# amirkdv/biseqt

Hardware: AMD Instinct MI355X
Metric: GCUPS (DP cell updates/s) banded local align (higher is better)
Workload: dtype i16

## Files before the change

biseqt_amd/csrc/pw_device.h:

```cpp
#ifndef PW_DEVICE_H
#define PW_DEVICE_H

#include <hip/hip_runtime.h>
#include <stdint.h>

#define PW_FN __device__ __forceinline__
#include "pw_wave.h"
#include "pw_launch.h"

namespace pw {

PW_FN uint32_t dev_shl1_in(uint32_t m, bool flag) {
  const uint64_t mask = __builtin_amdgcn_ballot_w64(flag);
  uint32_t r;
  uint64_t cout;
  asm("v_addc_co_u32 %0, %1, %2, %2, %3" : "=v"(r), "=s"(cout) : "v"(m), "s"(mask));
  return r;
}

template <typename T, bool ALWAYS_LDS> PW_FN T dev_tab_read(const T* tab, uint32_t handle, uint32_t off, bool in_lds) {
  typedef __attribute__((address_space(3))) const T lds_T;
  if (ALWAYS_LDS || in_lds) return *(lds_T*)(uintptr_t)(handle + off);
  return *(const T*)((const char*)tab + off);
}
PW_FN uint32_t dev_lds_handle(const void* p) {
  return (uint32_t)(uintptr_t)(__attribute__((address_space(3))) const char*)p;
}

PW_FN uint32_t dev_const_dword(const uint8_t* base, int idx) {
  typedef const __attribute__((address_space(4))) uint32_t c_u32;
  return ((c_u32*)base)[idx];
}

struct DevP {
  PW_FN static uint32_t const_dword(const uint8_t* base, int idx) { return dev_const_dword(base, idx); }
  template <typename T, bool A> PW_FN static T tab_read(const T* tab, uint32_t h, uint32_t off, bool in_lds) { return dev_tab_read<T, A>(tab, h, off, in_lds); }
  PW_FN static uint32_t shl1_in(uint32_t m, bool flag) { return dev_shl1_in(m, flag); }
  PW_FN static int lane() { return (int)(threadIdx.x & 63u); }
  PW_FN static int32_t shr1(int32_t v, int32_t old) {
    return __builtin_amdgcn_update_dpp(old, v, 0x138 , 0xf, 0xf, false);
  }
  PW_FN static int32_t shl1(int32_t v, int32_t old) {
    return __builtin_amdgcn_update_dpp(old, v, 0x130 , 0xf, 0xf, false);
  }
  PW_FN static int32_t shr1z(int32_t v) { return __builtin_amdgcn_update_dpp(0, v, 0x138 , 0xf, 0xf, true); }
  PW_FN static int32_t shl1z(int32_t v) { return __builtin_amdgcn_update_dpp(0, v, 0x130 , 0xf, 0xf, true); }
  PW_FN static int32_t shfl_xor(int32_t v, int m) { return __shfl_xor(v, m, 64); }
  PW_FN static int32_t uniform(int32_t v) { return __builtin_amdgcn_readfirstlane(v); }
  PW_FN static int nlanes() { return 64; }
  PW_FN static int nwaves() { return 1; }
  PW_FN static int32_t wave_bcast(int32_t v, int) { return v; }
  PW_FN static int lane0() { return 0; }
  PW_FN static bool central() { return true; }
  static constexpr bool kVirtualLanes = false;
  static constexpr bool kBatchedShifts = false;
};

template <int N, int MAXW> PW_FN void wg_shift_right(int32_t* v, const int32_t* old, int phase) {
  __shared__ int32_t edge[2][MAXW][N];
  const int w = (int)(threadIdx.x >> 6), l = (int)(threadIdx.x & 63u);
  int32_t r[N];
#pragma unroll
  for (int i = 0; i < N; i++) r[i] = __builtin_amdgcn_update_dpp(old[i], v[i], 0x138 , 0xf, 0xf, false);
  if (l == 63) {
#pragma unroll
    for (int i = 0; i < N; i++) edge[phase][w][i] = v[i];
  }
  asm volatile("s_waitcnt lgkmcnt(0)\n\ts_barrier" ::: "memory");
  if (l == 0 && w > 0) {
#pragma unroll
    for (int i = 0; i < N; i++) r[i] = edge[phase][w - 1][i];
  }
#pragma unroll
  for (int i = 0; i < N; i++) v[i] = r[i];
}
template <int N, int MAXW> PW_FN void wg_shift_left(int32_t* v, const int32_t* old, int phase) {
  __shared__ int32_t edge[2][MAXW][N];
  const int w = (int)(threadIdx.x >> 6), l = (int)(threadIdx.x & 63u), nw = (int)(blockDim.x >> 6);
  int32_t r[N];
#pragma unroll
  for (int i = 0; i < N; i++) r[i] = __builtin_amdgcn_update_dpp(old[i], v[i], 0x130 , 0xf, 0xf, false);
  if (l == 0) {
#pragma unroll
    for (int i = 0; i < N; i++) edge[phase][w][i] = v[i];
  }
  asm volatile("s_waitcnt lgkmcnt(0)\n\ts_barrier" ::: "memory");
  if (l == 63 && w + 1 < nw) {
#pragma unroll
    for (int i = 0; i < N; i++) r[i] = edge[phase][w + 1][i];
  }
#pragma unroll
  for (int i = 0; i < N; i++) v[i] = r[i];
}

struct DevPM {
  PW_FN static uint32_t const_dword(const uint8_t* base, int idx) { return dev_const_dword(base, idx); }
  template <typename T, bool A> PW_FN static T tab_read(const T* tab, uint32_t h, uint32_t off, bool in_lds) { return dev_tab_read<T, A>(tab, h, off, in_lds); }
  PW_FN static uint32_t shl1_in(uint32_t m, bool flag) { return dev_shl1_in(m, flag); }
  PW_FN static int lane() { return (int)threadIdx.x; }
  PW_FN static int lane0() { return 0; }
  PW_FN static bool central() { return true; }
  static constexpr bool kVirtualLanes = false;
  static constexpr bool kBatchedShifts = true;
  template <int N> PW_FN static void shrv(int32_t* v, const int32_t* old, int phase) { wg_shift_right<N, 16>(v, old, phase); }
  template <int N> PW_FN static void shlv(int32_t* v, const int32_t* old, int phase) { wg_shift_left<N, 16>(v, old, phase); }
  PW_FN static int nlanes() { return (int)blockDim.x; }
  PW_FN static int nwaves() { return (int)(blockDim.x >> 6); }
  PW_FN static int32_t shr1(int32_t v, int32_t old) {
    __shared__ int32_t edge[16];
    const int w = (int)(threadIdx.x >> 6), l = (int)(threadIdx.x & 63u);
    int32_t r = __builtin_amdgcn_update_dpp(old, v, 0x138 , 0xf, 0xf, false);
    if (l == 63) edge[w] = v;
    __syncthreads();
    if (l == 0 && w > 0) r = edge[w - 1];
    __syncthreads();
    return r;
  }
  PW_FN static int32_t shl1(int32_t v, int32_t old) {
    __shared__ int32_t edge[16];
    const int w = (int)(threadIdx.x >> 6), l = (int)(threadIdx.x & 63u);
    int32_t r = __builtin_amdgcn_update_dpp(old, v, 0x130 , 0xf, 0xf, false);
    if (l == 0) edge[w] = v;
    __syncthreads();
    if (l == 63 && w + 1 < (int)(blockDim.x >> 6)) r = edge[w + 1];
    __syncthreads();
    return r;
  }
  PW_FN static int32_t shfl_xor(int32_t v, int m) { return __shfl_xor(v, m, 64); }
  PW_FN static int32_t uniform(int32_t v) { return __builtin_amdgcn_readfirstlane(v); }
  PW_FN static int32_t wave_bcast(int32_t v, int w) {
    __shared__ int32_t slot[16];
    if ((threadIdx.x & 63u) == 0) slot[threadIdx.x >> 6] = v;
    __syncthreads();
    const int32_t r = slot[w];
    __syncthreads();
    return r;
  }
};

constexpr int kMaxLdsL = 32;

#ifndef PW_FILL_ATTR
#define PW_FILL_ATTR
#endif
template <typename T, int BK, bool BANY, bool TRACK, bool GENERIC>
__global__ __launch_bounds__(64) PW_FILL_ATTR void k_fill(const FillParams<T> a) {
  constexpr bool TAB = true;
  __shared__ T sub_lds[TAB ? kMaxLdsL * kMaxLdsL : 1];
  const T* tab = a.subst;
  if (TAB) {
    if (a.L <= kMaxLdsL) {
      for (int i = (int)threadIdx.x; i < a.L * a.L; i += 64) sub_lds[i] = a.subst[i];
      __syncthreads();
      tab = sub_lds;
    }
  }
  const int slot = (int)blockIdx.x;
  const int pair = a.order ? a.order[slot] : slot;
  const PairDesc pd = a.pairs[pair];
  WaveFill<DevP, T, BK, BANY, TRACK, GENERIC> w(a, pd, tab);
  w.tab_handle = dev_lds_handle(sub_lds); w.tab_in_lds = tab == sub_lds;
  w.pair_slot = pair;
  w.run();
}

#ifndef PW_FILL16_WAVES
#define PW_FILL16_WAVES 0
#endif
#ifndef PW_FILL16_WAVES_SEG
#define PW_FILL16_WAVES_SEG 0
#endif
template <int BK, bool SEG, int RULE> struct Fill16Occupancy {
  static constexpr unsigned w = SEG ? PW_FILL16_WAVES_SEG : PW_FILL16_WAVES;
  static constexpr unsigned lo = w ? w : 1, hi = w ? w : 8;
};
template <int BK, bool SEG, int RULE, bool MAT = false>
__global__ __launch_bounds__(64) PW_FILL_ATTR
__attribute__((amdgpu_waves_per_eu(Fill16Occupancy<BK, SEG, RULE>::lo, Fill16Occupancy<BK, SEG, RULE>::hi)))
void k_fill16(const FillParams<int32_t> a) {
  const WaveDesc wd = a.waves[blockIdx.x];
  WaveFill16<DevP, BK, SEG, RULE, MAT> w(a, wd);
  w.run();
}

template <int BK, int RULE, bool MAT = false>
__global__ __launch_bounds__(512) void k_fill16_mw(const FillParams<int32_t> a) {
  const WaveDesc wd = a.waves[blockIdx.x];
  WaveFill16<DevPM, BK, false, RULE, MAT> w(a, wd);
  w.run();
}

constexpr int kTileLanes = PW_TILE_LANES, kTileGhost = PW_TILE_GHOST, kTileCentral = kTileLanes - 2 * kTileGhost;
struct DevPT {
  PW_FN static uint32_t const_dword(const uint8_t* base, int idx) { return dev_const_dword(base, idx); }
  template <typename T, bool A> PW_FN static T tab_read(const T* tab, uint32_t h, uint32_t off, bool in_lds) { return dev_tab_read<T, A>(tab, h, off, in_lds); }
  PW_FN static uint32_t shl1_in(uint32_t m, bool flag) { return dev_shl1_in(m, flag); }
  PW_FN static int tile() {
#ifdef PW_TILE_NO_XCD_REMAP
    return (int)blockIdx.x;
#else
    return (int)(blockIdx.x & 7u) * (int)(gridDim.x >> 3) + (int)(blockIdx.x >> 3);
#endif
  }
  PW_FN static int lane0() { return tile() * kTileCentral - kTileGhost; }
  PW_FN static int lane() { return lane0() + (int)threadIdx.x; }
  PW_FN static int nlanes() { return lane0() + kTileLanes; }
  PW_FN static int nwaves() { return kTileLanes / 64; }
  PW_FN static bool central() { return (int)threadIdx.x >= kTileGhost && (int)threadIdx.x < kTileLanes - kTileGhost; }
  static constexpr bool kVirtualLanes = true;
  static constexpr bool kBatchedShifts = true;
  template <int N> PW_FN static void shrv(int32_t* v, const int32_t* old, int phase) { wg_shift_right<N, kTileLanes / 64>(v, old, phase); }
  template <int N> PW_FN static void shlv(int32_t* v, const int32_t* old, int phase) { wg_shift_left<N, kTileLanes / 64>(v, old, phase); }
  PW_FN static void wg_max4(int (&v)[4]) {
    __shared__ int red[4];
    if (threadIdx.x < 4) red[threadIdx.x] = -0x7fffffff;
    __syncthreads();
#pragma unroll
    for (int i = 0; i < 4; i++) atomicMax(&red[i], v[i]);
    __syncthreads();
#pragma unroll
    for (int i = 0; i < 4; i++) v[i] = red[i];
  }
  PW_FN static int32_t shr1(int32_t v, int32_t old) {
    __shared__ int32_t edge[kTileLanes / 64];
    const int w = (int)(threadIdx.x >> 6), l = (int)(threadIdx.x & 63u);
    int32_t r = __builtin_amdgcn_update_dpp(old, v, 0x138 , 0xf, 0xf, false);
    if (l == 63) edge[w] = v;
    __syncthreads();
    if (l == 0 && w > 0) r = edge[w - 1];
    __syncthreads();
    return r;
  }
  PW_FN static int32_t shl1(int32_t v, int32_t old) {
    __shared__ int32_t edge[kTileLanes / 64];
    const int w = (int)(threadIdx.x >> 6), l = (int)(threadIdx.x & 63u);
    int32_t r = __builtin_amdgcn_update_dpp(old, v, 0x130 , 0xf, 0xf, false);
    if (l == 0) edge[w] = v;
    __syncthreads();
    if (l == 63 && w + 1 < kTileLanes / 64) r = edge[w + 1];
    __syncthreads();
    return r;
  }
  PW_FN static int32_t shfl_xor(int32_t v, int m) { return __shfl_xor(v, m, 64); }
  PW_FN static int32_t uniform(int32_t v) { return __builtin_amdgcn_readfirstlane(v); }
  PW_FN static int32_t wave_bcast(int32_t v, int) { return v; }
};
// ... 138 lines not shown
```

biseqt_amd/csrc/pw_wave.h:

```cpp
#ifndef PW_WAVE_H
#define PW_WAVE_H

#ifndef PW_FN
#error "PW_FN must be defined by the includer"
#endif

#include "pw_types.h"
#if !defined(__HIPCC__)
#include <stdlib.h>
#endif

namespace pw {

template <typename T> struct ScoreTraits;
template <> struct ScoreTraits<int32_t> {
  static constexpr bool is_int = true;
  PW_FN static int32_t neg() { return -(1 << 28); }
  PW_FN static int32_t zero_blk() { return 0; }
  PW_FN static int32_t max2(int32_t a, int32_t b) { return a > b ? a : b; }
  PW_FN static int32_t gap_offer(bool kept, int32_t go, int32_t A) { return kept ? A : A + go; }
};
template <> struct ScoreTraits<double> {
  static constexpr bool is_int = false;
  PW_FN static double neg() { return -1.0e300; }
// ... 452 lines not shown
      const int ox = P::shfl_xor(cx, off), oy = P::shfl_xor(cy, off), oh = P::shfl_xor(hv, off);
      const bool take = oh && (!hv || os > cs || (os == cs && ok_ < ck));
      if (take) { cs = os; ck = ok_; cx = ox; cy = oy; hv = 1; }
    }
    if (P::nwaves() > 1) {
      T bs = cs; uint64_t bk_ = ck; int bx = cx, by = cy, bh = 0;
      for (int wv = 0; wv < P::nwaves(); wv++) {
        const T os = xwave_bcast<P>(cs, wv);
        const uint64_t ok_ = xwave_bcast<P>(ck, wv);
        const int ox = P::wave_bcast(cx, wv), oy = P::wave_bcast(cy, wv), oh = P::wave_bcast(hv, wv);
        const bool take = oh && (!bh || os > bs || (os == bs && ok_ < bk_));
        if (take) { bs = os; bk_ = ok_; bx = ox; by = oy; bh = 1; }
      }
      cs = bs; ck = bk_; cx = bx; cy = by; hv = bh;
    }
    if (lane == 0) {
      Result r;
      r.score = (double)cs * a.score_mul;
      r.opt_i = a.banded ? cx - cy - pd.dmin : cx;
      r.opt_j = a.banded ? (cx < cy ? cx : cy) : cy;
      r.origin_idx = 0; r.mutant_idx = 0; r.tx_len = 0; r.status = 0;
      if (!hv || (endrule == END_STD_LOCAL && !(cs > T(0)))) { r.opt_i = -1; r.opt_j = -1; r.score = 0.0; }
      a.results[pair_slot] = r;
    }
  }
  int pair_slot;
};

struct __attribute__((aligned(8))) U4 { uint32_t x, y, z, w; };
struct __attribute__((packed)) PackedU64 { uint64_t v; };
struct __attribute__((packed)) PackedU32 { uint32_t v; };

namespace pk {
#if defined(__HIP_DEVICE_COMPILE__)
typedef short s2_t __attribute__((ext_vector_type(2)));
typedef unsigned short u2_t __attribute__((ext_vector_type(2)));
PW_FN s2_t as_s2(uint32_t v) { return __builtin_bit_cast(s2_t, v); }
PW_FN u2_t as_u2(uint32_t v) { return __builtin_bit_cast(u2_t, v); }
PW_FN uint32_t add(uint32_t a, uint32_t b) { return __builtin_bit_cast(uint32_t, (u2_t)(as_u2(a) + as_u2(b))); }
PW_FN uint32_t sub(uint32_t a, uint32_t b) { return __builtin_bit_cast(uint32_t, (u2_t)(as_u2(a) - as_u2(b))); }
PW_FN uint32_t add32(uint32_t a, uint32_t b) { return a + b; }
PW_FN uint32_t subsat(uint32_t a, uint32_t b) { return __builtin_bit_cast(uint32_t, __builtin_elementwise_sub_sat(as_u2(a), as_u2(b))); }
PW_FN uint32_t max(uint32_t a, uint32_t b) { return __builtin_bit_cast(uint32_t, __builtin_elementwise_max(as_s2(a), as_s2(b))); }
PW_FN uint32_t minu(uint32_t a, uint32_t b) { return __builtin_bit_cast(uint32_t, __builtin_elementwise_min(as_u2(a), as_u2(b))); }
PW_FN uint32_t maxu(uint32_t a, uint32_t b) { return __builtin_bit_cast(uint32_t, __builtin_elementwise_max(as_u2(a), as_u2(b))); }
PW_FN uint32_t shru(uint32_t a, uint32_t sh) { return __builtin_bit_cast(uint32_t, (u2_t)(as_u2(a) >> as_u2(sh))); }
PW_FN uint32_t mad(uint32_t a, uint32_t b, uint32_t c) { return __builtin_bit_cast(uint32_t, (u2_t)(as_u2(a) * as_u2(b) + as_u2(c))); }
PW_FN uint32_t mins(uint32_t a, uint32_t b) { return __builtin_bit_cast(uint32_t, __builtin_elementwise_min(as_s2(a), as_s2(b))); }
PW_FN uint32_t align16(uint32_t hi, uint32_t lo) { return __builtin_amdgcn_alignbit(hi, lo, 16); }
PW_FN uint32_t sign(uint32_t a, uint32_t sh15) { return __builtin_bit_cast(uint32_t, (s2_t)(as_s2(a) >> as_s2(sh15))); }
PW_FN uint32_t opaque(uint32_t v) { asm volatile("" : "+v"(v)); return v; }
PW_FN uint32_t opaque_su(uint32_t v) { asm volatile("" : "+s"(v)); return v; }
PW_FN uint8_t* opaque_s(uint8_t* v) { asm volatile("" : "+s"(v)); return v; }
PW_FN void store_global(uint8_t* base, uint32_t off, const U4& v) {
  typedef __attribute__((address_space(1))) uint8_t gbyte_t;
  typedef __attribute__((address_space(1))) U4 gu4_t;
  *(gu4_t*)((gbyte_t*)base + off) = v;
}
PW_FN uint32_t perm(uint32_t a, uint32_t b, uint32_t sel) { return __builtin_amdgcn_perm(a, b, sel); }
#else
PW_FN uint32_t mk(uint32_t lo, uint32_t hi) { return (lo & 0xffffu) | (hi << 16); }
PW_FN int32_t sl(uint32_t v) { return (int16_t)(v & 0xffffu); }
PW_FN int32_t sh(uint32_t v) { return (int16_t)(v >> 16); }
PW_FN uint32_t add(uint32_t a, uint32_t b) { return mk((a & 0xffffu) + (b & 0xffffu), (a >> 16) + (b >> 16)); }
PW_FN uint32_t sub(uint32_t a, uint32_t b) { return mk((a & 0xffffu) - (b & 0xffffu), (a >> 16) - (b >> 16)); }
#if !defined(__HIPCC__)
inline unsigned& add32_breaches() { static unsigned n = 0; return n; }
PW_FN uint32_t add32(uint32_t a, uint32_t b) {
  if ((a & 0xffffu) >= 0xff80u || (a >> 16) >= 0xff80u) add32_breaches()++;
  return a + b;
}
#else
PW_FN uint32_t add32(uint32_t a, uint32_t b) { return a + b; }
#endif
PW_FN uint32_t subsat(uint32_t a, uint32_t b) {
  const uint32_t al = a & 0xffffu, bl = b & 0xffffu, ah = a >> 16, bh = b >> 16;
  return mk(al > bl ? al - bl : 0u, ah > bh ? ah - bh : 0u);
}
PW_FN uint32_t max(uint32_t a, uint32_t b) { return mk((uint32_t)(sl(a) > sl(b) ? sl(a) : sl(b)), (uint32_t)(sh(a) > sh(b) ? sh(a) : sh(b))); }
PW_FN uint32_t minu(uint32_t a, uint32_t b) {
  const uint32_t al = a & 0xffffu, bl = b & 0xffffu, ah = a >> 16, bh = b >> 16;
  return mk(al < bl ? al : bl, ah < bh ? ah : bh);
}
PW_FN uint32_t mad(uint32_t a, uint32_t b, uint32_t c) {
  return mk((uint32_t)(sl(a) * sl(b) + sl(c)), (uint32_t)(sh(a) * sh(b) + sh(c)));
}
PW_FN uint32_t maxu(uint32_t a, uint32_t b) {
  const uint32_t al = a & 0xffffu, bl = b & 0xffffu, ah = a >> 16, bh = b >> 16;
  return mk(al > bl ? al : bl, ah > bh ? ah : bh);
}
PW_FN uint32_t shru(uint32_t a, uint32_t sh) { return mk((a & 0xffffu) >> (sh & 0xfu), (a >> 16) >> ((sh >> 16) & 0xfu)); }
PW_FN uint32_t mins(uint32_t a, uint32_t b) { return mk((uint32_t)(sl(a) < sl(b) ? sl(a) : sl(b)), (uint32_t)(sh(a) < sh(b) ? sh(a) : sh(b))); }
PW_FN uint32_t align16(uint32_t hi, uint32_t lo) { return (lo >> 16) | (hi << 16); }
PW_FN uint32_t sign(uint32_t a, uint32_t) { return mk(sl(a) < 0 ? 0xffffu : 0u, sh(a) < 0 ? 0xffffu : 0u); }
PW_FN uint32_t opaque(uint32_t v) { return v; }
PW_FN uint32_t opaque_su(uint32_t v) { return v; }
PW_FN uint8_t* opaque_s(uint8_t* v) { return v; }
PW_FN void store_global(uint8_t* base, uint32_t off, const U4& v) { *(U4*)(base + off) = v; }
PW_FN uint32_t perm(uint32_t a, uint32_t b, uint32_t sel) {
  const uint64_t in = ((uint64_t)a << 32) | b;
  uint32_t r = 0;
  for (int i = 0; i < 4; i++) {
    const uint32_t c = (sel >> (8 * i)) & 0xffu;
    uint32_t v;
    if (c >= 13) v = 0xffu;
    else if (c == 12) v = 0u;
    else if (c >= 8) v = ((in >> (8 * (2 * (c - 8) + 1) + 7)) & 1u) ? 0xffu : 0u;
    else v = (uint32_t)(in >> (8 * c)) & 0xffu;
    r |= v << (8 * i);
  }
  return r;
}
#endif
PW_FN uint32_t both(int32_t v) { return ((uint32_t)v & 0xffffu) | ((uint32_t)v << 16); }
PW_FN uint32_t pack(int32_t lo, int32_t hi) { return ((uint32_t)lo & 0xffffu) | ((uint32_t)hi << 16); }
PW_FN int32_t lo_s(uint32_t v) { return (int32_t)(int16_t)(v & 0xffffu); }
PW_FN int32_t hi_s(uint32_t v) { return (int32_t)(int16_t)(v >> 16); }
}
#if !defined(__HIPCC__)
extern "C" __attribute__((used, visibility("default"))) inline unsigned pw_pk_add32_breaches(int reset) {
  const unsigned n = pk::add32_breaches();
  if (reset) pk::add32_breaches() = 0;
  return n;
}
namespace pk {
inline unsigned* ramp_block_counts() { static unsigned n[4] = {0, 0, 0, 0}; return n; }
inline int& ramp_free_emu() { static int v = -1; return v; }
}
extern "C" __attribute__((used, visibility("default"))) inline void pw_ramp_block_counts(unsigned* out, int reset) {
  for (int i = 0; i < 4; i++) { out[i] = pk::ramp_block_counts()[i]; if (reset) pk::ramp_block_counts()[i] = 0; }
}
extern "C" __attribute__((used, visibility("default"))) inline void pw_emu_ramp_free(int v) { pk::ramp_free_emu() = v; }
#endif

template <class P, int BK, bool SEG, int RULE = 0, bool MAT = false>
struct WaveFill16 {
  static constexpr bool SC4 = RULE == 3;
  static constexpr int RL = SC4 ? 0 : RULE;
  static constexpr int SCL = SC4 ? 4 : 1;
  static constexpr bool ANYB = RL == 0 || RL == 4;
  static constexpr bool TRK = RL == 0 || RL == 5;
  static constexpr bool CAP = !TRK;
  static_assert(BK % 4 == 0, "packed layout needs an even number of cells per step");
  static constexpr int R = BK / 2;
  static constexpr int RH = R / 2;
#ifdef PW_FILL16_UNR
  static constexpr int UNR = PW_FILL16_UNR;
#else
  static constexpr int UNR = BK <= 8 ? 4 : (BK <= 16 ? 2 : 1);
#endif
  static constexpr int32_t NEG16 = ANYB ? -8192 : -24000;
  static constexpr uint32_t SENT_O = 0xfffeu, SENT_M = 0xffffu;
  static constexpr uint32_t MSEL = 0x0c00u, MOUT = 8u;
  static constexpr bool FIXSEL = MAT && RH == 2;
  PW_FN static uint32_t sel4_fed(int it) { return ((uint32_t)it >> 1) & 1u; }
  PW_FN static bool sel4_lo(int k, int p) { return (((k + 7 - p) >> 1) & 1) != 0; }
  using Base = WaveFill<P, int32_t, BK, true, true, false>;

  const FillParams<int32_t>& a;
  const WaveDesc wd;
  PairDesc pd;
  int li;
  bool valid, segfirst, seglast;
  int pair_slot;
  const uint8_t* oseq;
  const uint8_t* mseq;
  int X, Y, ndiag, owlast, mwlast, xfeed_o, yfeed_m;
  uint32_t fo_lo, fo_hi, fm_lo, fm_hi, fo_n0, fo_n1, fo_n2, fm_n0, fm_n1, fm_n2;

  uint32_t HE[RH], UE[RH], LE[RH], HO[RH], UO[RH], LO[RH];
  uint32_t bestE[RH], bestO[RH], btE[RH], btO[RH];
  uint32_t gebE[RH], gebO[RH];
  uint32_t clE[RH], clO[RH];
  uint32_t tfE[RH], tfO[RH], tlE[RH], tlO[RH];
  uint32_t accE[RH], accO[RH], acc2E[RH], acc2O[RH];
  uint32_t OW[RH], MW[RH];
  uint32_t ROW[MAT ? R : 1];
  uint32_t BIASV, MADJ;
  uint32_t MR0, MR1, MR2, MR3;
  uint32_t ONE, SH15, C2, C4, C16, NDELTA, MATCHV, GOV, GOVI, NEGV, LIMV;
  uint32_t kbE[RH], kbO[RH], C8, SEVEN;
  uint32_t up_prev;
  uint32_t left_next;
  int phase_l, phase_r;
  uint32_t mrow0, mrow_step, mspare, mgroup;
  static constexpr bool SPLIT = ANYB && MAT;
  static constexpr bool KEPT = SC4 && SPLIT;
  static constexpr bool SBASE = !SEG && SPLIT;
  static constexpr bool RAMPF = SPLIT && TRK;
  bool rf;
  uint32_t flimx, flimy;
  uint32_t mrowb;
  uint8_t* mbase[BK / 4];

  PW_FN WaveFill16(const FillParams<int32_t>& a_, const WaveDesc& wd_) : a(a_), wd(wd_) {}

  template <int EK>
  PW_FN void cellpair(uint32_t& Hs, uint32_t& Us, uint32_t& Ls, uint32_t& bests, uint32_t& bts, uint32_t geb,
                      uint32_t tf, uint32_t tl, uint32_t& acc, uint32_t up, uint32_t left, uint32_t oc,
                      uint32_t mc, uint32_t tv, uint32_t clampL = 0, uint32_t och = 0, bool lo4 = false) {
    constexpr bool EDGE = EK != 0;
    uint32_t hM;
    constexpr bool FLOOR0 = MAT && ANYB && (EK & 1) == 0;
    if (MAT) {
      const uint32_t sub2 = lo4 ? pk::perm(oc, och, mc) : pk::perm(och, oc, mc);
      const uint32_t hb = ANYB ? pk::add32(Hs, sub2) : pk::add(Hs, sub2);
      hM = FLOOR0 ? pk::subsat(hb, BIASV) : pk::sub(hb, BIASV);
    } else {
      const uint32_t ne = pk::minu(oc ^ mc, ONE);
      hM = pk::add(Hs, pk::mad(ne, NDELTA, MATCHV));
    }
    uint32_t Hn = pk::max(pk::max(up, left), hM);
    uint32_t nB;
    if (ANYB) {
      if (EK & 1) Hn = pk::max(Hn, pk::sign(pk::sub(tv, tf), SH15) & NEGV);
      else if (!FLOOR0) Hn = pk::max(Hn, 0u);
      nB = KEPT ? pk::subsat(ONE, Hn) : pk::minu(Hn, ONE);
    } else {
      const uint32_t Bc = EDGE ? pk::mad(pk::minu(tv ^ tf, ONE), NEGV, 0u) : NEGV;
      Hn = pk::max(Hn, Bc);
      nB = pk::minu(Hn ^ Bc, ONE);
    }
    const uint32_t nD = KEPT ? pk::subsat(C2, Hn ^ up) : pk::minu(Hn ^ up, SC4 ? C2 : ONE);
    const uint32_t nI = KEPT ? pk::subsat(C4, Hn ^ left) : pk::minu(Hn ^ left, SC4 ? C4 : ONE);
    const uint32_t hg = pk::add(Hn, geb);
    Us = pk::mad(nD, GOV, hg);
    Ls = pk::mad(nI, GOVI, hg);
    if (!ANYB) Ls = pk::mins(Ls, clampL);
    if (SC4) acc = pk::mad(acc, C16, nB + nD + nI);
    else acc = pk::mad(acc, C16, pk::mad(nI, C4, pk::mad(nD, C2, nB)));
    if (TRK) {
    } else if (EK & 2) {
      const uint32_t e = pk::minu(tv ^ tl, ONE);
      bests = pk::mad(e, pk::sub(bests, Hn), Hn);
    }
    Hs = Hn;
  }

  PW_FN void stamp_best(uint32_t& bts, uint32_t kb, uint32_t kb0, uint32_t blk8) {
    const uint32_t ch = pk::minu((kb ^ kb0) & ~SEVEN, ONE);
    bts = pk::maxu(bts, pk::mad(ch, blk8, kb & SEVEN));
  }

  template <int EK>
  PW_FN void track_key(uint32_t& kb, uint32_t H, uint32_t tl, uint32_t tv, int k) {
    const uint32_t hk = (!ANYB || (EK & 1)) ? pk::max(H, 0u) : H;
    uint32_t key = pk::mad(hk, SC4 ? C2 : C8, pk::both(7 - k));
    if (EK & 2) key &= ~pk::sign(pk::sub(tl, tv), SH15);
    kb = pk::maxu(kb, key);
  }

  template <int EK, int HALF>
  PW_FN void iteration16(int it, int k) {
    constexpr bool EDGE = EK != 0;
    const uint32_t tv0 = pk::both(2 * it), tv1 = pk::both(2 * it + 1);
    {
      uint32_t prev = up_prev;
      if (SEG) prev = segfirst ? NEGV : prev;
      const uint32_t up0 = pk::align16(UO[RH - 1], prev);
#pragma unroll
      for (int p = 0; p < RH; p++)
      {
        cellpair<EK>(HE[p], UE[p], LE[p], bestE[p], btE[p], gebE[p], tfE[p], tlE[p], HALF == 0 ? accE[p] : acc2E[p],
                     p == 0 ? up0 : UO[p == 0 ? 0 : p - 1], LO[p], MAT ? ROW[MAT ? p : 0] : OW[p], MW[p], tv0, clE[p],
                     MAT ? ROW[MAT ? p + RH : 0] : 0u, FIXSEL && sel4_lo(k, p));
        if (TRK) track_key<EK>(kbE[p], HE[p], tlE[p], tv0, k);
      }
    }
    {
      const int oi = xfeed_o + it;
      const uint32_t fb = Base::feed_byte(fo_lo, fo_hi, k);
      uint32_t feed = (!EDGE || (uint32_t)oi < (uint32_t)X) ? fb : SENT_O;
      if (MAT) feed = row_of(fb);
      int32_t mv[2] = {(int32_t)(MAT ? ROW[0] : OW[0]), (int32_t)LE[0]};
      const int32_t mo[2] = {(int32_t)feed, (int32_t)left_next};
      xshlv<P, 2>(mv, mo, phase_l); phase_l ^= 1;
      uint32_t nxt = (uint32_t)mv[0];
      left_next = (uint32_t)mv[1];
      if (SEG) nxt = seglast ? feed : nxt;
      if (MAT) {
#pragma unroll
        for (int i = 0; i + 1 < (MAT ? R : 1); i++) ROW[i] = ROW[i + 1];
        ROW[MAT ? R - 1 : 0] = nxt;
      } else {
        const uint32_t last = pk::align16(nxt, OW[0]);
#pragma unroll
        for (int p = 0; p + 1 < RH; p++) OW[p] = OW[p + 1];
        OW[RH - 1] = last;
      }
    }
    {
      uint32_t nxt = left_next;
      if (SEG) nxt = seglast ? NEGV : nxt;
      const uint32_t leftl = pk::align16(nxt, LE[0]);
#pragma unroll
      for (int p = 0; p < RH; p++)
      {
        cellpair<EK>(HO[p], UO[p], LO[p], bestO[p], btO[p], gebO[p], tfO[p], tlO[p], HALF == 0 ? accO[p] : acc2O[p],
                     UE[p], p == RH - 1 ? leftl : LE[p == RH - 1 ? p : p + 1], MAT ? ROW[MAT ? p : 0] : OW[p], MW[p], tv1, clO[p],
                     MAT ? ROW[MAT ? p + RH : 0] : 0u, FIXSEL && sel4_lo(k, p));
        if (TRK) track_key<EK>(kbO[p], HO[p], tlO[p], tv1, k);
      }
    }
    {
      const int mi = yfeed_m + it;
      const uint32_t fbm = Base::feed_byte(fm_lo, fm_hi, k);
      const uint32_t feed = (MAT ? (MSEL | (fbm + 4u * (FIXSEL ? sel4_fed(k) : 1u)))
                                 : ((!EDGE || (uint32_t)mi < (uint32_t)Y) ? fbm : SENT_M)) << 16;
      int32_t mv[2] = {(int32_t)MW[RH - 1], (int32_t)UO[RH - 1]};
      const int32_t mo[2] = {(int32_t)feed, (int32_t)up_prev};
      xshrv<P, 2>(mv, mo, phase_r); phase_r ^= 1;
      uint32_t prv = (uint32_t)mv[0];
      up_prev = (uint32_t)mv[1];
      if (SEG) prv = segfirst ? feed : prv;
      uint32_t first = pk::align16(MW[RH - 1], prv);
      if (MAT && !FIXSEL) first += MADJ;
#pragma unroll
      for (int p = RH - 1; p > 0; p--) MW[p] = MW[p - 1];
      MW[0] = first;
    }
  }

  template <int EK>
  PW_FN void block16(int b) {
#if !defined(__HIPCC__)
    if (P::lane() == 0) pk::ramp_block_counts()[EK]++;
#endif
#pragma unroll
    for (int p = 0; p < RH; p++) { accE[p] = 0; accO[p] = 0; acc2E[p] = 0; acc2O[p] = 0; }
    uint32_t kb0E[RH], kb0O[RH];
    if (TRK) {
#pragma unroll
      for (int p = 0; p < RH; p++) { kb0E[p] = kbE[p]; kb0O[p] = kbO[p]; }
    }
#pragma clang loop unroll_count(UNR)
    for (int k = 0; k < 4; k++) iteration16<EK, 0>(8 * b + k, k);
#pragma clang loop unroll_count(UNR)
    for (int k = 4; k < 8; k++) iteration16<EK, 1>(8 * b + k, k);
    if (TRK) {
      const uint32_t blk8 = pk::both(8 * b + 8);
#pragma unroll
      for (int p = 0; p < RH; p++) {
        stamp_best(btE[p], kbE[p], kb0E[p], blk8);
        stamp_best(btO[p], kbO[p], kb0O[p], blk8);
      }
    }
    {
      uint32_t mwd[BK];
#pragma unroll
      for (int p = 0; p < RH; p++) {
        const uint32_t inv = KEPT ? 0u : 0x77777777u;
        const uint32_t kE = KEPT ? accE[p] : inv - accE[p], k2E = KEPT ? acc2E[p] : inv - acc2E[p];
        const uint32_t kO = KEPT ? accO[p] : inv - accO[p], k2O = KEPT ? acc2O[p] : inv - acc2O[p];
        mwd[2 * p] = pk::perm(kE, k2E, 0x05040100u);
        mwd[2 * p + R] = pk::perm(kE, k2E, 0x07060302u);
        mwd[2 * p + 1] = pk::perm(kO, k2O, 0x05040100u);
        mwd[2 * p + 1 + R] = pk::perm(kO, k2O, 0x07060302u);
      }
      if (!SBASE) {
        const uint32_t row = b < pd.nblocks ? mrow0 + (uint32_t)b * mrow_step : mspare;
        uint32_t* dst = a.masks + pd.mask_off;
#pragma unroll
        for (int g = 0; g < BK / 4; g++) {
          U4 v; v.x = mwd[4 * g]; v.y = mwd[4 * g + 1]; v.z = mwd[4 * g + 2]; v.w = mwd[4 * g + 3];
          *(U4*)(dst + (row + (uint32_t)g * mgroup)) = v;
        }
      } else {
#pragma unroll
        for (int g = 0; g < BK / 4; g++) {
          U4 v; v.x = mwd[4 * g]; v.y = mwd[4 * g + 1]; v.z = mwd[4 * g + 2]; v.w = mwd[4 * g + 3];
          pk::store_global(mbase[g], mrowb, v);
        }
        mrowb += 4u * mrow_step;
      }
    }
  }

  PW_FN void feed_issue(int b) {
    const uint32_t* o32 = (const uint32_t*)oseq;
    const uint32_t* m32 = (const uint32_t*)mseq;
    const int wo = (xfeed_o + 8 * b) >> 2, wm = (yfeed_m + 8 * b) >> 2;
    if (!SEG) {
      fo_n0 = P::const_dword(oseq, pw_clampi(wo, 0, owlast)); fo_n1 = P::const_dword(oseq, pw_clampi(wo + 1, 0, owlast));
      fo_n2 = P::const_dword(oseq, pw_clampi(wo + 2, 0, owlast));
      fm_n0 = P::const_dword(mseq, pw_clampi(wm, 0, mwlast)); fm_n1 = P::const_dword(mseq, pw_clampi(wm + 1, 0, mwlast));
      fm_n2 = P::const_dword(mseq, pw_clampi(wm + 2, 0, mwlast));
      return;
    }
    fo_n0 = o32[pw_clampi(wo, 0, owlast)]; fo_n1 = o32[pw_clampi(wo + 1, 0, owlast)]; fo_n2 = o32[pw_clampi(wo + 2, 0, owlast)];
    fm_n0 = m32[pw_clampi(wm, 0, mwlast)]; fm_n1 = m32[pw_clampi(wm + 1, 0, mwlast)]; fm_n2 = m32[pw_clampi(wm + 2, 0, mwlast)];
  }
  PW_FN static int clamp08(int v) {
    if (SEG) return pw_clampi(v, 0, 8);
    const int r = (int)pk::opaque_su((uint32_t)(v > 0 ? v : 0));
    return r < 8 ? r : 8;
  }
  PW_FN static uint64_t inside_bytes(int i0, int n) {
    const int lo = clamp08(-i0), hi = clamp08(n - i0);
    const uint64_t below_hi = hi >= 8 ? ~(uint64_t)0 : (((uint64_t)1 << (8 * hi)) - 1);
    const uint64_t below_lo = lo >= 8 ? ~(uint64_t)0 : (((uint64_t)1 << (8 * lo)) - 1);
    return below_hi & ~below_lo;
  }
  template <bool RT = false>
  PW_FN void feed_commit(int b, bool edge) {
    const int ro = (xfeed_o + 8 * b) & 3, rm = (yfeed_m + 8 * b) & 3;
    fo_lo = Base::funnel(fo_n1, fo_n0, ro); fo_hi = Base::funnel(fo_n2, fo_n1, ro);
    fm_lo = Base::funnel(fm_n1, fm_n0, rm); fm_hi = Base::funnel(fm_n2, fm_n1, rm);
    if (MAT && edge) {
      const uint64_t io = inside_bytes(xfeed_o + 8 * b, X), im = inside_bytes(yfeed_m + 8 * b, Y);
      const uint64_t o = ((((uint64_t)fo_hi) << 32) | fo_lo) | ~io;
      const uint64_t m = (((((uint64_t)fm_hi) << 32) | fm_lo) & im) | ((0x0101010101010101ull * MOUT) & ~im);
      fo_lo = (uint32_t)o; fo_hi = (uint32_t)(o >> 32);
      fm_lo = (uint32_t)m; fm_hi = (uint32_t)(m >> 32);
      if (!SEG && !RT) { fo_hi = pk::opaque_su(fo_hi); fm_hi = pk::opaque_su(fm_hi); }
    }
    if (MAT && !SEG && RT) { fo_hi = pk::opaque_su(fo_hi); fm_hi = pk::opaque_su(fm_hi); }
  }

  PW_FN int tfirst_of(int j) const {
    const int dd = li * BK + j, d = pd.dmin + dd;
    if (MAT && ANYB && valid && dd == ndiag) return 0;
    return (valid && dd < ndiag) ? (d < 0 ? -d : d) - pd.s0 : 32767;
  }
  PW_FN int tlast_of(int j) const {
    const int dd = li * BK + j, d = pd.dmin + dd;
    if (!valid || dd >= ndiag) return -1;
    const int len = 1 + (d > 0 ? 0 : d) + (X - d > Y ? Y : X - d);
    return (d < 0 ? -d : d) - pd.s0 + 2 * (len - 1);
  }
  PW_FN int tbegin_of(int j) const {
    const int dd = li * BK + j, d = pd.dmin + dd;
    if (!valid || dd >= ndiag) return 32767;
    if ((RL == 2 || RL == 5 || a.brule == BRULE_ORIGIN) && d != 0) return 32767;
    return (d < 0 ? -d : d) - pd.s0;
  }
  PW_FN uint32_t row_of(uint32_t l) const {
    uint32_t r = l == 3u ? MR3 : 0u;
    r = l == 2u ? MR2 : r;
    r = l == 1u ? MR1 : r;
    return l == 0u ? MR0 : r;
  }
  PW_FN uint32_t row_at(int i) const { return (uint32_t)i < (uint32_t)X ? row_of((uint32_t)oseq[i]) : 0u; }
  PW_FN uint32_t msel(int i, uint32_t plus4) const { return MSEL | (((uint32_t)i < (uint32_t)Y ? (uint32_t)mseq[i] : MOUT) + 4u * plus4); }
  PW_FN uint32_t letter_o(int i) const { return (uint32_t)i < (uint32_t)X ? (uint32_t)oseq[i] : SENT_O; }
  PW_FN uint32_t letter_m(int i) const { return (uint32_t)i < (uint32_t)Y ? (uint32_t)mseq[i] : SENT_M; }
  PW_FN int blocked(int j) const { return li * BK + j == ndiag ? NEG16 : 0; }
  PW_FN int start_of(int j) const { return (valid && li * BK + j <= ndiag) ? 0 : NEG16; }
  PW_FN bool ramp_free_on() const {
#if !defined(__HIPCC__)
    if (pk::ramp_free_emu() >= 0) {
      const char* knob = getenv("PWLIB_RAMP_BLOCKS");
      return pk::ramp_free_emu() != 0 && !(knob && atoi(knob) != 0);
    }
#endif
    return a.ramp_free != 0;
  }

  PW_FN void run() {
    const int lane = P::lane();
    const int nl = wd.nl;
    const int seg = lane / nl;
    li = lane - seg * nl;
    valid = seg < wd.count;
    segfirst = li == 0; seglast = li == nl - 1;
    const int slot = wd.first + ((SEG && valid) ? seg : 0);
    pair_slot = a.order ? a.order[slot] : slot;
    if (!SEG) pair_slot = P::uniform(pair_slot);
    pd = a.pairs[pair_slot];
    X = pd.X; Y = pd.Y; ndiag = pd.ndiag;
    oseq = a.arena + pd.o_off; mseq = a.arena + pd.m_off;
    owlast = (X > 0 ? X - 1 : 0) >> 2; mwlast = (Y > 0 ? Y - 1 : 0) >> 2;
    const int e = (pd.s0 + pd.dmin) >> 1;
    const int f = (pd.s0 - pd.dmin) >> 1;
    const int xbase = e + li * R, ybase = f - li * R;
    xfeed_o = e + nl * R - 1;
    yfeed_m = f;
    rf = RAMPF && ramp_free_on();
    ONE = pk::opaque(0x00010001u); SH15 = pk::opaque(0x000f000fu);
    C2 = pk::opaque(0x00020002u); C4 = pk::opaque(0x00040004u); C16 = pk::opaque(0x00100010u);
    C8 = pk::opaque(0x00080008u); SEVEN = pk::opaque(0x00070007u);
    NEGV = pk::both(NEG16); LIMV = pk::both(-32767);
    NDELTA = pk::both(SCL * (a.mismatch - a.match)); MATCHV = pk::both(SCL * a.match);
    GOV = pk::both(KEPT ? -2 * a.go : (SC4 ? 2 * a.go : a.go)); GOVI = pk::both(KEPT ? -a.go : a.go);
    BIASV = pk::both(a.mat_bias); MADJ = 0x0003fffcu;
    MR0 = a.mat_rows[0]; MR1 = a.mat_rows[1]; MR2 = a.mat_rows[2]; MR3 = a.mat_rows[3];
    if (MAT) {
#pragma unroll
      for (int i = 0; i < (MAT ? R : 1); i++) ROW[i] = row_at(xbase + i - 1);
    }
#pragma unroll
    for (int p = 0; p < RH; p++) {
      const int e0 = 2 * p, e1 = 2 * p + R, o0 = 2 * p + 1, o1 = 2 * p + 1 + R;
      if (ANYB) {
        const int geo = SCL * a.ge + (KEPT ? SCL * a.go : 0);
        gebE[p] = pk::pack(geo + blocked(e0), geo + blocked(e1));
        gebO[p] = pk::pack(geo + blocked(o0), geo + blocked(o1));
        tfE[p] = pk::pack(tfirst_of(e0), tfirst_of(e1)); tfO[p] = pk::pack(tfirst_of(o0), tfirst_of(o1));
        clE[p] = clO[p] = 0;
      } else {
        gebE[p] = gebO[p] = pk::both(a.ge);
        clE[p] = pk::pack(blocked(e0) ? NEG16 : 32767, blocked(e1) ? NEG16 : 32767);
        clO[p] = pk::pack(blocked(o0) ? NEG16 : 32767, blocked(o1) ? NEG16 : 32767);
        tfE[p] = pk::pack(tbegin_of(e0), tbegin_of(e1)); tfO[p] = pk::pack(tbegin_of(o0), tbegin_of(o1));
      }
      tlE[p] = pk::pack(tlast_of(e0), tlast_of(e1)); tlO[p] = pk::pack(tlast_of(o0), tlast_of(o1));
      HE[p] = UE[p] = LE[p] = HO[p] = UO[p] = LO[p] = NEGV;
      if (RAMPF && rf) {
        HE[p] = pk::pack(start_of(e0), start_of(e1)); HO[p] = pk::pack(start_of(o0), start_of(o1));
      }
      up_prev = left_next = NEGV; phase_l = 0; phase_r = 0;
      bestE[p] = bestO[p] = NEGV;
      kbE[p] = kbO[p] = 0u; btE[p] = btO[p] = 0u;
      OW[p] = pk::pack((int32_t)letter_o(xbase + p - 1), (int32_t)letter_o(xbase + p + RH - 1));
      if (MAT) {
        const int yl = ybase - p - 1, yh = ybase - p - RH - 1;
        MW[p] = pk::pack((int32_t)msel(yl, FIXSEL ? sel4_fed(yl - f) : 0u), (int32_t)msel(yh, FIXSEL ? sel4_fed(yh - f) : 1u));
      }
      else MW[p] = pk::pack((int32_t)letter_m(ybase - p - 1), (int32_t)letter_m(ybase - p - RH - 1));
    }
    const int sb1 = CAP ? wd.steady_b1 - 1 : wd.steady_b1;
    mgroup = 4u * (uint32_t)pd.nl;
    mspare = (uint32_t)mask_word_index(BK, pd.nl, pd.nblocks, 0, 0);
    const bool mrow_ok = valid && li < pd.nl;
    mrow0 = mrow_ok ? (uint32_t)mask_word_index(BK, pd.nl, 0, li, 0) : mspare;
    mrow_step = mrow_ok ? (uint32_t)mask_word_index(BK, pd.nl, 1, 0, 0) : 0u;
    mrowb = 4u * mrow0;
    if (SBASE) {
#pragma unroll
      for (int g = 0; g < BK / 4; g++)
        mbase[g] = pk::opaque_s((uint8_t*)(a.masks + pd.mask_off) + (uint64_t)(4u * (uint32_t)g * mgroup));
    }
    feed_issue(0);
    if constexpr (SPLIT) {
      const int nb = nblocks_run();
      const int b0 = wd.steady_b0 < nb ? (wd.steady_b0 > 0 ? wd.steady_b0 : 0) : nb;
      const int b1 = sb1 < nb ? sb1 : nb;
      const int r0 = (RAMPF && rf) ? 0 : b0, r1 = (RAMPF && rf) ? nb : b1;
      flimx = (uint32_t)(X > 7 ? X - 7 : 0); flimy = (uint32_t)(Y > 7 ? Y - 7 : 0);
      int b = 0;
      if (sb1 > wd.steady_b0) for (; b < r0; b++) blocks_step<1>(b);
      else for (; b < r0; b++) blocks_step<3>(b);
      for (; b < r1; b++) blocks_step<0>(b);
      for (; b < nb; b++) blocks_step<2>(b);
    } else {
      for (int b = 0, nb = nblocks_run(); b < nb; b++) {
        const bool steady = b >= wd.steady_b0 && b < sb1;
        feed_commit(b, !steady);
        if (b + 1 < nb) feed_issue(b + 1);
        if (steady) block16<0>(b);
        else if (!ANYB) block16<3>(b);
        else if (b >= wd.steady_b0) block16<2>(b);
        else if (sb1 > wd.steady_b0) block16<1>(b);
        else block16<3>(b);
      }
    }
    finish();
  }
  PW_FN int nblocks_run() const { return SBASE ? (wd.nblocks < pd.nblocks ? wd.nblocks : pd.nblocks) : wd.nblocks; }
  template <int EK>
  PW_FN void blocks_step(int b) {
    if constexpr (RAMPF && EK == 0)
      feed_commit<true>(b, rf & (((uint32_t)(xfeed_o + 8 * b) >= flimx) | ((uint32_t)(yfeed_m + 8 * b) >= flimy)));
    else feed_commit(b, EK != 0);
    if (b + 1 < nblocks_run()) feed_issue(b + 1);
    block16<EK>(b);
  }

  PW_FN void finish() {
    const int endrule = a.endrule;
    int32_t cs = -32768; uint64_t ck = ~(uint64_t)0; int cx = -1, cy = -1; bool have = false;
    uint32_t parked[4 * RH];
#pragma unroll
    for (int p = 0; p < RH; p++) {
      parked[4 * p] = TRK ? pk::opaque(kbE[p]) : bestE[p]; parked[4 * p + 1] = TRK ? pk::opaque(btE[p]) : 0u;
      parked[4 * p + 2] = TRK ? pk::opaque(kbO[p]) : bestO[p]; parked[4 * p + 3] = TRK ? pk::opaque(btO[p]) : 0u;
    }
#pragma unroll 1
    for (int q = 0; q < 2 * RH; q++) {
      const int p = q >> 1, odd = q & 1;
      const uint32_t bq = parked[4 * p + 2 * odd], tq = parked[4 * p + 2 * odd + 1];
#pragma unroll 1
      for (int h = 0; h < 2; h++) {
        const int j = 2 * p + odd + h * R;
        const int dd = li * BK + j, d = pd.dmin + dd;
        const int tfirst = (d < 0 ? -d : d) - pd.s0;
// ... 170 lines not shown
```

Measured before the change: 2799.

## Stream sequence feed with sliding dword window and precomputed matrix rows

For non-segmented waves, the sequence feed keeps a sliding window and fetches only two new dwords per block with a single scalar 64-bit constant load, instead of three clamped scalar loads per sequence. Near the sequence ends it falls back to a clamped late reload. For the matrix-scoring path with small blocks, the eight feed rows are computed once per block in feed_commit instead of per step. This aims to cut scalar load and address arithmetic on the critical loop, at the cost of more bookkeeping state and registers, plus new host-emulation counters for boundary breaches.

```diff
diff --git a/biseqt_amd/csrc/pw_device.h b/biseqt_amd/csrc/pw_device.h
--- a/biseqt_amd/csrc/pw_device.h
+++ b/biseqt_amd/csrc/pw_device.h
@@ -32,7 +32,18 @@
   return ((c_u32*)base)[idx];
 }
 
-struct DevP {
+typedef uint64_t FeedDwords __attribute__((aligned(4)));
+PW_FN uint64_t dev_const_dword2(const uint8_t* base, uint32_t byte_off) {
+  typedef const __attribute__((address_space(4))) uint8_t c_u8;
+  typedef const __attribute__((address_space(4))) FeedDwords c_fd;
+  return *(c_fd*)((c_u8*)base + byte_off + 4u);
+}
+
+struct DevFeed {
+  PW_FN static uint64_t const_dword2(const uint8_t* base, uint32_t byte_off) { return dev_const_dword2(base, byte_off); }
+};
+
+struct DevP : DevFeed {
   PW_FN static uint32_t const_dword(const uint8_t* base, int idx) { return dev_const_dword(base, idx); }
   template <typename T, bool A> PW_FN static T tab_read(const T* tab, uint32_t h, uint32_t off, bool in_lds) { return dev_tab_read<T, A>(tab, h, off, in_lds); }
   PW_FN static uint32_t shl1_in(uint32_t m, bool flag) { return dev_shl1_in(m, flag); }
@@ -93,7 +104,7 @@
   for (int i = 0; i < N; i++) v[i] = r[i];
 }
 
-struct DevPM {
+struct DevPM : DevFeed {
   PW_FN static uint32_t const_dword(const uint8_t* base, int idx) { return dev_const_dword(base, idx); }
   template <typename T, bool A> PW_FN static T tab_read(const T* tab, uint32_t h, uint32_t off, bool in_lds) { return dev_tab_read<T, A>(tab, h, off, in_lds); }
   PW_FN static uint32_t shl1_in(uint32_t m, bool flag) { return dev_shl1_in(m, flag); }
@@ -191,7 +202,7 @@
 }
 
 constexpr int kTileLanes = PW_TILE_LANES, kTileGhost = PW_TILE_GHOST, kTileCentral = kTileLanes - 2 * kTileGhost;
-struct DevPT {
+struct DevPT : DevFeed {
   PW_FN static uint32_t const_dword(const uint8_t* base, int idx) { return dev_const_dword(base, idx); }
   template <typename T, bool A> PW_FN static T tab_read(const T* tab, uint32_t h, uint32_t off, bool in_lds) { return dev_tab_read<T, A>(tab, h, off, in_lds); }
   PW_FN static uint32_t shl1_in(uint32_t m, bool flag) { return dev_shl1_in(m, flag); }
diff --git a/biseqt_amd/csrc/pw_wave.h b/biseqt_amd/csrc/pw_wave.h
--- a/biseqt_amd/csrc/pw_wave.h
+++ b/biseqt_amd/csrc/pw_wave.h
@@ -528,6 +528,11 @@
 PW_FN uint32_t opaque(uint32_t v) { asm volatile("" : "+v"(v)); return v; }
 PW_FN uint32_t opaque_su(uint32_t v) { asm volatile("" : "+s"(v)); return v; }
 PW_FN uint8_t* opaque_s(uint8_t* v) { asm volatile("" : "+s"(v)); return v; }
+PW_FN uint32_t copy_su(uint32_t src, uint32_t& pass) {
+  uint32_t d;
+  asm volatile("s_mov_b32 %0, %2" : "=&s"(d), "+s"(pass) : "s"(src));
+  return d;
+}
 PW_FN void store_global(uint8_t* base, uint32_t off, const U4& v) {
   typedef __attribute__((address_space(1))) uint8_t gbyte_t;
   typedef __attribute__((address_space(1))) U4 gu4_t;
@@ -572,6 +577,7 @@
 PW_FN uint32_t opaque(uint32_t v) { return v; }
 PW_FN uint32_t opaque_su(uint32_t v) { return v; }
 PW_FN uint8_t* opaque_s(uint8_t* v) { return v; }
+PW_FN uint32_t copy_su(uint32_t src, uint32_t&) { return src; }
 PW_FN void store_global(uint8_t* base, uint32_t off, const U4& v) { *(U4*)(base + off) = v; }
 PW_FN uint32_t perm(uint32_t a, uint32_t b, uint32_t sel) {
   const uint64_t in = ((uint64_t)a << 32) | b;
@@ -607,6 +613,18 @@
   for (int i = 0; i < 4; i++) { out[i] = pk::ramp_block_counts()[i]; if (reset) pk::ramp_block_counts()[i] = 0; }
 }
 extern "C" __attribute__((used, visibility("default"))) inline void pw_emu_ramp_free(int v) { pk::ramp_free_emu() = v; }
+namespace pk {
+inline unsigned& feed_breaches() { static unsigned n = 0; return n; }
+inline unsigned* feed_path_counts() { static unsigned n[4] = {0, 0, 0, 0}; return n; }
+}
+extern "C" __attribute__((used, visibility("default"))) inline unsigned pw_feed_breaches(int reset) {
+  const unsigned n = pk::feed_breaches();
+  if (reset) pk::feed_breaches() = 0;
+  return n;
+}
+extern "C" __attribute__((used, visibility("default"))) inline void pw_feed_path_counts(unsigned* out, int reset) {
+  for (int i = 0; i < 4; i++) { out[i] = pk::feed_path_counts()[i]; if (reset) pk::feed_path_counts()[i] = 0; }
+}
 #endif
 
 template <class P, int BK, bool SEG, int RULE = 0, bool MAT = false>
@@ -642,7 +660,9 @@
   const uint8_t* oseq;
   const uint8_t* mseq;
   int X, Y, ndiag, owlast, mwlast, xfeed_o, yfeed_m;
-  uint32_t fo_lo, fo_hi, fm_lo, fm_hi, fo_n0, fo_n1, fo_n2, fm_n0, fm_n1, fm_n2;
+  uint32_t fo_lo, fo_hi, fm_lo, fm_hi, fo_n0, fm_n0;
+  uint64_t fo_n12, fm_n12;
+  uint32_t fo_w, fm_w, fo_lim, fm_lim;
 
   uint32_t HE[RH], UE[RH], LE[RH], HO[RH], UO[RH], LO[RH];
   uint32_t bestE[RH], bestO[RH], btE[RH], btO[RH];
@@ -664,6 +684,8 @@
   static constexpr bool KEPT = SC4 && SPLIT;
   static constexpr bool SBASE = !SEG && SPLIT;
   static constexpr bool RAMPF = SPLIT && TRK;
+  static constexpr bool FROWS = MAT && !SEG && UNR == 4 && BK <= 8;
+  uint32_t frow[FROWS ? 8 : 1];
   bool rf;
   uint32_t flimx, flimy;
   uint32_t mrowb;
@@ -747,7 +769,7 @@
       const int oi = xfeed_o + it;
       const uint32_t fb = Base::feed_byte(fo_lo, fo_hi, k);
       uint32_t feed = (!EDGE || (uint32_t)oi < (uint32_t)X) ? fb : SENT_O;
-      if (MAT) feed = row_of(fb);
+      if (MAT) feed = FROWS ? frow[FROWS ? k : 0] : row_of(fb);
       int32_t mv[2] = {(int32_t)(MAT ? ROW[0] : OW[0]), (int32_t)LE[0]};
       const int32_t mo[2] = {(int32_t)feed, (int32_t)left_next};
       xshlv<P, 2>(mv, mo, phase_l); phase_l ^= 1;
@@ -852,19 +874,61 @@
     }
   }
 
+  PW_FN static uint64_t dwords(uint32_t lo, uint32_t hi) { return ((uint64_t)hi << 32) | lo; }
+  PW_FN static void feed_count(int which) {
+#if !defined(__HIPCC__)
+    if (P::lane() == 0) pk::feed_path_counts()[which]++;
+#endif
+  }
+  PW_FN static uint32_t feed_dword(const uint8_t* base, int idx, int wlast) {
+#if !defined(__HIPCC__)
+    if (idx < 0 || idx > wlast) { pk::feed_breaches()++; return 0xa5a5a5a5u; }
+#endif
+    return P::const_dword(base, idx);
+  }
+  PW_FN static uint64_t feed_dword2(const uint8_t* base, uint32_t byte_off, int wlast) {
+#if !defined(__HIPCC__)
+    const int idx = (int)(byte_off + 4u) >> 2;
+    if ((byte_off & 3u) != 0) pk::feed_breaches()++;
+    return dwords(feed_dword(base, idx, wlast), feed_dword(base, idx + 1, wlast));
+#else
+    return P::const_dword2(base, byte_off);
+#endif
+  }
+  PW_FN void feed_load3(const uint8_t* seq, int wlast, uint32_t fw, uint32_t& n0, uint64_t& n12) {
+    const int w = (int)fw >> 2;
+    n0 = feed_dword(seq, pw_clampi(w, 0, wlast), wlast);
+    n12 = dwords(feed_dword(seq, pw_clampi(w + 1, 0, wlast), wlast), feed_dword(seq, pw_clampi(w + 2, 0, wlast), wlast));
+  }
+  PW_FN void feed_late(const uint8_t* seq, int wlast, uint32_t fw, uint32_t& n0, uint64_t& n12, int which) {
+    const int w = (int)fw >> 2;
+    feed_count(2 * which + 1);
+    if (w >= wlast || w + 2 <= 0) { n0 = (uint32_t)(n12 >> 32); n12 = dwords(n0, n0); }
+    else feed_load3(seq, wlast, fw, n0, n12);
+  }
+  PW_FN void feed_ahead(const uint8_t* seq, int wlast, uint32_t& fw, uint32_t flim, uint32_t& n0, uint64_t& n12, int which) {
+    fw += 8u;
+    if (fw < flim) {
+      feed_count(2 * which);
+      n0 = pk::copy_su((uint32_t)(n12 >> 32), fw);
+      n12 = feed_dword2(seq, fw, wlast);
+    }
+  }
+  template <bool FIRST = false>
   PW_FN void feed_issue(int b) {
+    if (!SEG) {
+      if (FIRST) {
+        feed_load3(oseq, owlast, fo_w, fo_n0, fo_n12); feed_load3(mseq, mwlast, fm_w, fm_n0, fm_n12);
+      } else {
+        feed_ahead(oseq, owlast, fo_w, fo_lim, fo_n0, fo_n12, 0); feed_ahead(mseq, mwlast, fm_w, fm_lim, fm_n0, fm_n12, 1);
+      }
+      return;
+    }
     const uint32_t* o32 = (const uint32_t*)oseq;
     const uint32_t* m32 = (const uint32_t*)mseq;
     const int wo = (xfeed_o + 8 * b) >> 2, wm = (yfeed_m + 8 * b) >> 2;
-    if (!SEG) {
-      fo_n0 = P::const_dword(oseq, pw_clampi(wo, 0, owlast)); fo_n1 = P::const_dword(oseq, pw_clampi(wo + 1, 0, owlast));
-      fo_n2 = P::const_dword(oseq, pw_clampi(wo + 2, 0, owlast));
-      fm_n0 = P::const_dword(mseq, pw_clampi(wm, 0, mwlast)); fm_n1 = P::const_dword(mseq, pw_clampi(wm + 1, 0, mwlast));
-      fm_n2 = P::const_dword(mseq, pw_clampi(wm + 2, 0, mwlast));
-      return;
-    }
-    fo_n0 = o32[pw_clampi(wo, 0, owlast)]; fo_n1 = o32[pw_clampi(wo + 1, 0, owlast)]; fo_n2 = o32[pw_clampi(wo + 2, 0, owlast)];
-    fm_n0 = m32[pw_clampi(wm, 0, mwlast)]; fm_n1 = m32[pw_clampi(wm + 1, 0, mwlast)]; fm_n2 = m32[pw_clampi(wm + 2, 0, mwlast)];
+    fo_n0 = o32[pw_clampi(wo, 0, owlast)]; fo_n12 = dwords(o32[pw_clampi(wo + 1, 0, owlast)], o32[pw_clampi(wo + 2, 0, owlast)]);
+    fm_n0 = m32[pw_clampi(wm, 0, mwlast)]; fm_n12 = dwords(m32[pw_clampi(wm + 1, 0, mwlast)], m32[pw_clampi(wm + 2, 0, mwlast)]);
   }
   PW_FN static int clamp08(int v) {
     if (SEG) return pw_clampi(v, 0, 8);
@@ -880,17 +944,34 @@
   template <bool RT = false>
   PW_FN void feed_commit(int b, bool edge) {
     const int ro = (xfeed_o + 8 * b) & 3, rm = (yfeed_m + 8 * b) & 3;
-    fo_lo = Base::funnel(fo_n1, fo_n0, ro); fo_hi = Base::funnel(fo_n2, fo_n1, ro);
-    fm_lo = Base::funnel(fm_n1, fm_n0, rm); fm_hi = Base::funnel(fm_n2, fm_n1, rm);
+    if (!SEG) {
+      const bool late_o = fo_w >= fo_lim, late_m = fm_w >= fm_lim;
+      if (late_o | late_m) {
+        if (late_o) feed_late(oseq, owlast, fo_w, fo_n0, fo_n12, 0);
+        if (late_m) feed_late(mseq, mwlast, fm_w, fm_n0, fm_n12, 1);
+      }
+    }
+    fo_lo = Base::funnel((uint32_t)fo_n12, fo_n0, ro); fo_hi = (uint32_t)(fo_n12 >> (8 * ro));
+    fm_lo = Base::funnel((uint32_t)fm_n12, fm_n0, rm); fm_hi = (uint32_t)(fm_n12 >> (8 * rm));
+    if (FROWS) {
+#pragma unroll
+      for (int k = 0; k < 8; k++) frow[k] = row_bits(fo_lo, fo_hi, k);
+    }
     if (MAT && edge) {
       const uint64_t io = inside_bytes(xfeed_o + 8 * b, X), im = inside_bytes(yfeed_m + 8 * b, Y);
-      const uint64_t o = ((((uint64_t)fo_hi) << 32) | fo_lo) | ~io;
       const uint64_t m = (((((uint64_t)fm_hi) << 32) | fm_lo) & im) | ((0x0101010101010101ull * MOUT) & ~im);
-      fo_lo = (uint32_t)o; fo_hi = (uint32_t)(o >> 32);
       fm_lo = (uint32_t)m; fm_hi = (uint32_t)(m >> 32);
-      if (!SEG && !RT) { fo_hi = pk::opaque_su(fo_hi); fm_hi = pk::opaque_su(fm_hi); }
-    }
-    if (MAT && !SEG && RT) { fo_hi = pk::opaque_su(fo_hi); fm_hi = pk::opaque_su(fm_hi); }
+      if (FROWS) {
+        const uint32_t io_lo = pk::opaque_su((uint32_t)io), io_hi = pk::opaque_su((uint32_t)(io >> 32));
+#pragma unroll
+        for (int k = 0; k < 8; k++) frow[k] = (((k < 4 ? io_lo : io_hi) >> (8 * (k & 3))) & 1u) ? frow[k] : 0u;
+      } else {
+        const uint64_t o = ((((uint64_t)fo_hi) << 32) | fo_lo) | ~io;
+        fo_lo = (uint32_t)o; fo_hi = (uint32_t)(o >> 32);
+      }
+      if (!SEG && !RT) { if (!FROWS) fo_hi = pk::opaque_su(fo_hi); fm_hi = pk::opaque_su(fm_hi); }
+    }
+    if (MAT && !SEG && RT) { if (!FROWS) fo_hi = pk::opaque_su(fo_hi); fm_hi = pk::opaque_su(fm_hi); }
   }
 
   PW_FN int tfirst_of(int j) const {
@@ -915,6 +996,12 @@
     r = l == 2u ? MR2 : r;
     r = l == 1u ? MR1 : r;
     return l == 0u ? MR0 : r;
+  }
+  PW_FN uint32_t row_bits(uint32_t lo, uint32_t hi, int k) const {
+    const uint32_t w = k < 4 ? lo : hi;
+    const bool b0 = (w & (1u << (8 * (k & 3)))) != 0, b1 = (w & (2u << (8 * (k & 3)))) != 0;
+    const uint32_t r01 = b0 ? MR1 : MR0, r23 = b0 ? MR3 : MR2;
+    return b1 ? r23 : r01;
   }
   PW_FN uint32_t row_at(int i) const { return (uint32_t)i < (uint32_t)X ? row_of((uint32_t)oseq[i]) : 0u; }
   PW_FN uint32_t msel(int i, uint32_t plus4) const { return MSEL | (((uint32_t)i < (uint32_t)Y ? (uint32_t)mseq[i] : MOUT) + 4u * plus4); }
@@ -951,6 +1038,8 @@
     const int xbase = e + li * R, ybase = f - li * R;
     xfeed_o = e + nl * R - 1;
     yfeed_m = f;
+    fo_w = (uint32_t)xfeed_o & ~3u; fm_w = (uint32_t)yfeed_m & ~3u;
+    fo_lim = 4u * (uint32_t)(owlast > 1 ? owlast - 1 : 0); fm_lim = 4u * (uint32_t)(mwlast > 1 ? mwlast - 1 : 0);
     rf = RAMPF && ramp_free_on();
     ONE = pk::opaque(0x00010001u); SH15 = pk::opaque(0x000f000fu);
     C2 = pk::opaque(0x00020002u); C4 = pk::opaque(0x00040004u); C16 = pk::opaque(0x00100010u);
@@ -1006,7 +1095,7 @@
       for (int g = 0; g < BK / 4; g++)
         mbase[g] = pk::opaque_s((uint8_t*)(a.masks + pd.mask_off) + (uint64_t)(4u * (uint32_t)g * mgroup));
     }
-    feed_issue(0);
+    feed_issue<true>(0);
     if constexpr (SPLIT) {
       const int nb = nblocks_run();
       const int b0 = wd.steady_b0 < nb ? (wd.steady_b0 > 0 ? wd.steady_b0 : 0) : nb;
```

New measurement: 2858 (median of 6 runs). 1.02x the previous value.
